# DaDaMrX/ReaLiSe

Measured on AMD Instinct MI355X. Metric: train sentences/sec (seq_len=128), higher is better.
Workload: dtype bf16

## Files before the change

### realise_amd/csrc/capi.hip

```cpp
#include <math.h>
#include <string.h>

#include "attention.h"
#include "engine.h"
#include "gemm.h"
#include "layout.h"
#include "ops.h"
#include "prof.h"
#include "../../include/realise_hip_debug.h"

using namespace rl;
#define RL_TRY(expr) do { const int _rc = (expr); if (_rc != RL_OK) return _rc; } while (0)

struct realise_engine { EngineBase* impl; };

namespace {
template <typename T> EpiParams<T> to_epi(const realise_epilogue* e) {
  EpiParams<T> p;
  if (!e) return p;
  p.mode = e->mode; p.accumulate = e->accumulate; p.out = (T*)e->out; p.ldo = e->ldo; p.out2 = (T*)e->out2;
  p.bias = e->bias; p.aux = (const T*)e->aux; p.ldaux = e->ldaux; p.alpha = e->alpha;
  p.drop_seed = e->drop_seed; p.drop_thresh = e->drop_thresh; p.drop_scale = e->drop_scale;
  return p;
}
// ... 124 lines not shown
  if (live == nullptr || n_live == nullptr) return RL_ERR_ARG;
  if (dtype == REALISE_BF16) return tn_grouped<bf16_t>(st, n, problems, P, live, n_live, list_rows, overwrite);
  if (dtype == REALISE_F32) return tn_grouped<float>(st, n, problems, P, live, n_live, list_rows, overwrite);
  return RL_ERR_ARG;
}
int realise_conv_tn(void* stream, int dtype, const void* A, int64_t lda, const realise_conv_geom* b, int P, int Co, int Ci,
                    float* out, float* scratch, int64_t scratch_elems) {
  hipStream_t st = (hipStream_t)stream;
  if (!b) return RL_ERR_ARG;
  TnEpi te; te.mode = TN_CONVW; te.out = out; te.Cin = Ci; te.Cpad = b->C; te.KHW = b->KH * b->KW;
  te.slab = scratch; te.slab_elems = scratch_elems;
  const int J = b->KH * b->KW * b->C;
  if (dtype == REALISE_BF16) return gemm_tn_conv<bf16_t>(st, (const bf16_t*)A, lda, to_geom<bf16_t>(b), P, Co, J, te);
  if (dtype == REALISE_F32) return gemm_tn_conv<float>(st, (const float*)A, lda, to_geom<float>(b), P, Co, J, te);
  return RL_ERR_ARG;
}
void realise_set_tn_transpose_read(int enable) { set_tn_transpose_read(enable); }
void realise_set_nt_allow_n96(int on) { set_nt_allow_n96(on); }
void realise_set_nt_variant(int v) { set_nt_variant(v); }
void realise_set_nt_group_m(int g) { set_nt8_group_m(g); }
void realise_set_ln(int key, int value) {
  if (key == 0) set_ln_fast(value); else if (key == 1) set_ln_bwd_blocks(value); else if (key == 2) set_bn_fast(value); else if (key == 3) set_bn_chunks(value); else if (key == 4) set_ce_fast(value); else if (key == 5) set_ln_v2(value); else if (key == 6) set_adamw_reg(value);
}
void realise_set_engine(int key, int value) { if (key == 0) set_fwd_order(value); else if (key >= 1 && key <= 3) set_stream_priority(key - 1, value); else if (key == 4) set_cls_compact(value); else if (key == 5) set_skip_dead(value); else if (key == 6) set_cls_splitk(value); else if (key == 9) set_gru_fuse(value); else if (key == 10) set_live_rows(value); else if (key == 13) set_glyph_fuse(value); else if (key == 14) set_bn_fold(value); else if (key == 15) set_opt_pipe(value); }
void realise_set_nt8p(int key, int value) { if (key == 0) set_nt8p_order(value); else if (key == 1) set_nt8p_wgs(value); else if (key == 3) set_nt8_live_gc(value); }
void realise_set_tn_split(int n) { set_tn_split(n); }
void realise_set_wgrad_group(int on) { set_wgrad_group(on); }
void realise_set_dgrad_parity(int on) { set_dgrad_parity(on); }
void realise_set_conv_c64(int on) { set_conv_c64(on); }
void realise_set_glyph_dedup(int on) { set_glyph_dedup(on); }
void realise_set_wgrad_overlap(int on) { set_wgrad_overlap(on); }
void realise_set_branch_overlap(int on) { set_branch_overlap(on); }

int realise_attention_fwd(void* stream, int dtype, const void* q, const void* k, const void* v, int64_t ldq, const float* mask_add,
                          void* ctx, int64_t ldc, float* lse, int B, int nh, int S, uint32_t drop_seed, uint32_t drop_thresh,
                          float drop_scale) {
  hipStream_t st = (hipStream_t)stream;
  if (dtype == REALISE_BF16)
    return attn_fwd<bf16_t>(st, (const bf16_t*)q, (const bf16_t*)k, (const bf16_t*)v, ldq, mask_add, (bf16_t*)ctx, ldc, lse, B, nh, S,
                            drop_seed, drop_thresh, drop_scale);
  if (dtype == REALISE_F32)
    return attn_fwd<float>(st, (const float*)q, (const float*)k, (const float*)v, ldq, mask_add, (float*)ctx, ldc, lse, B, nh, S,
                           drop_seed, drop_thresh, drop_scale);
  return RL_ERR_ARG;
}
int realise_attention_bwd(void* stream, int dtype, const void* q, const void* k, const void* v, int64_t ldq, const float* mask_add,
                          const void* ctx, const void* dctx, int64_t ldc, const float* lse, float* rowdot, void* dq, void* dk,
// ... 411 lines not shown
```

### realise_amd/csrc/engine.h

```cpp
#pragma once
#include <hip/hip_runtime.h>
#include <stdint.h>
#include "../../include/realise_hip.h"

namespace rl {
struct AdamwGroups;
void set_wgrad_overlap(int on);
void set_wgrad_group(int on);
void set_dgrad_parity(int on);
void set_fwd_order(int o);
void set_skip_dead(int on);
void set_cls_compact(int on);
void set_gru_fuse(int on);
void set_glyph_fuse(int on);
void set_opt_pipe(int on);
void set_bn_fold(int on);
void set_live_rows(int on);
void set_cls_splitk(int n);
void set_stream_priority(int which, int pri);
void set_branch_overlap(int on);

struct EngineBase {
  virtual ~EngineBase() {}
  virtual int64_t shadow_bytes() const = 0;
  virtual int64_t workspace_bytes(int B, int S, int Tp) = 0;
  virtual int bind(void* shadow, void* workspace, int64_t bytes) = 0;
  virtual void forget_workspace(void* workspace) = 0;
  virtual int64_t plan_install_count() const = 0;
  virtual int refresh_shadows(hipStream_t st) = 0;
  virtual int refresh_shadows_ex(hipStream_t st, int skip_linear) = 0;
  virtual int adamw_step(hipStream_t st, float* m, float* v, const uint8_t* group_of_block, const struct AdamwGroups& gs, const float* norm_sq,
                         float max_norm, int pipelined) = 0;
  virtual int sync_optimizer(hipStream_t st) = 0;
  virtual void invalidate_frozen() = 0;
  virtual void set_id_flag(int* flag) = 0;
  virtual void set_grads_fresh(int fresh) = 0;
  virtual void set_loss_grad(const float* grad_dev) = 0;
  virtual int forward(hipStream_t st, const realise_batch& b) = 0;
// ... 9 lines not shown
```

### realise_amd/csrc/engine.hip

```cpp
#include <math.h>
#include <stdio.h>
#include <string.h>
#include <algorithm>
#include <map>
#include <string>
#include <vector>

#include "attention.h"
#include "engine.h"
#include "gemm.h"
#include "layout.h"
#include "ops.h"

namespace rl {

static int g_wgrad_overlap = 1;
void set_wgrad_overlap(int on) { g_wgrad_overlap = on; }
static int g_wgrad_group = 1;
void set_wgrad_group(int on) { g_wgrad_group = on; }
static int g_dgrad_parity = 1;
void set_dgrad_parity(int on) { g_dgrad_parity = on; }
static int g_branch_overlap = 1;
void set_branch_overlap(int on) { g_branch_overlap = on; }
static int g_fwd_order = 0;
void set_fwd_order(int o) { g_fwd_order = o; }
static int g_skip_dead = 1;
void set_skip_dead(int on) { g_skip_dead = on; }
static int g_cls_compact = 1;
void set_cls_compact(int on) { g_cls_compact = on; }
static int g_gru_fuse = 1;
void set_gru_fuse(int on) { g_gru_fuse = on; }
static int g_cls_splitk = 3;
void set_cls_splitk(int n) { g_cls_splitk = n < 0 ? 0 : (n > 4 ? 4 : n); }
static int g_live_rows = 2;
void set_live_rows(int on) { g_live_rows = on; }
static int g_glyph_fuse = 1;
void set_glyph_fuse(int on) { g_glyph_fuse = on; }
static int g_bn_fold = 1;
void set_bn_fold(int on) { g_bn_fold = on; }
static int g_opt_pipe = 1;
void set_opt_pipe(int on) { g_opt_pipe = on; }
static int g_stream_pri[3] = {0, 0, 0};
void set_stream_priority(int which, int pri) { if (which >= 0 && which < 3) g_stream_pri[which] = pri < 0 ? -1 : (pri > 0 ? 1 : 0); }
static hipError_t create_stream(hipStream_t* s, int which) {
  if (g_stream_pri[which] == 0) return hipStreamCreateWithFlags(s, hipStreamNonBlocking);
  int least = 0, greatest = 0;
  if (hipDeviceGetStreamPriorityRange(&least, &greatest) != hipSuccess) return hipStreamCreateWithFlags(s, hipStreamNonBlocking);
  return hipStreamCreateWithPriority(s, hipStreamNonBlocking, g_stream_pri[which] < 0 ? greatest : least);
}

#define RL_TRY(expr) do { const int _rc = (expr); if (_rc != RL_OK) { fprintf(stderr, "[realise_hip] %s failed (%d) at %s:%d\n", #expr, _rc, __FILE__, __LINE__); return _rc; } } while (0)

static constexpr int64_t TN_SLAB_ELEMS = 16LL << 20;
static inline int64_t al256(int64_t x) { return (x + 255) & ~(int64_t)255; }
struct Bump {
  int64_t off = 0;
  int64_t take(int64_t bytes) { const int64_t o = off; off = al256(off + bytes); return o; }
};

static inline uint64_t splitmix(uint64_t x) {
  x += 0x9E3779B97F4A7C15ull;
  x = (x ^ (x >> 30)) * 0xBF58476D1CE4E5B9ull;
  x = (x ^ (x >> 27)) * 0x94D049BB133111EBull;
  return x ^ (x >> 31);
}

template <typename T> struct Engine : EngineBase {
  realise_config cfg;
  Variant vr;
  Layout L;
  float *P = nullptr, *G = nullptr, *PU = nullptr, *FZ = nullptr, *BF = nullptr;
  int64_t* BI = nullptr;
  char* sh = nullptr;
  char* ws = nullptr;
  int64_t ws_bytes = 0;
  int H, nh, I, V;
  int Vp;

  struct LayerSh { int64_t qkv_w, qkv_wT, ao_w, ao_wT, in_w, in_wT, out_w, out_wT; };
  struct BlockSh { int64_t w1f, w1d, w1p, w2f, w2d, wsf, wsd; int cin_pad; };
  std::vector<LayerSh> sh_bert, sh_pho, sh_out;
  BlockSh sh_blk[TOWER_MAX_BLOCKS];
  int64_t sh_cls_w = 0, sh_cls_wT = 0, sh_gru_hh = 0, sh_gru_hhT = 0, sh_glyph = 0;
  int64_t sh_head_w = 0, sh_head_wT = 0;
  int64_t shadow_total = 0;
  bool glyph_built = false, descs_built = false;
  int64_t sh_descs = 0, sh_fill = 0, sh_skip = 0;
  bool skip_built = false;
  static constexpr int ACHUNK_MAX = 8192, ACHUNK_LEN = 32768;
  std::vector<FillChunk> achunk_host;
  int n_achunks = 0;
  static constexpr int FILL_MAX = 2048;
  int n_descs = 0, desc_tiles = 0;
  std::vector<CastDesc> desc_host;

  struct LayerAct { int64_t qkv, lse, ctx, s1, rstd1, y1, pre, post, s2, rstd2, y2; };
  struct StackAct { int64_t emb_y, emb_xhat, emb_rstd; std::vector<LayerAct> layers; };
  struct BnAct { int64_t mean, rstd, scale, shift; };
  struct BlockAct { int64_t c1, h1, c2, cs, out; BnAct bn1, bn2, bns; int Hin, Hout, Pout; };
  struct Plan {
    int B = 0, S = 0, Tp = 0;
    int64_t total = 0;
    StackAct bert, pho, outb;
    BlockAct blk[TOWER_MAX_BLOCKS];
    int64_t mask_add, out_d, dlogits, count, loss_internal;
    int64_t cls_act, cls_inv, cls_nact, cls_xc, cls_gc, cls_slab;
    int64_t live_rows = 0;
    int64_t row_live, live_t64, live_t32, live_t16, live_n, live_rlen;
    int64_t ids_clean = 0, pho_clean = 0;
    int64_t gru_table, gru_hs, gru_rzn, gru_gh, gru_out;
    int64_t res_xhat, res_rstd, res_h, gate_mean, gate_msum, gate_g, fused;
// ... 164 lines not shown
    };
    auto add_stack = [&](const StackOff& so, const std::vector<LayerSh>& v) {
      for (size_t l = 0; l < v.size(); ++l) {
        const LayerOff& o = so.layers[l];
        add(o.qkv_w, 3 * H, H, v[l].qkv_w, v[l].qkv_wT);
        add(o.ao_w, H, H, v[l].ao_w, v[l].ao_wT);
        add(o.in_w, I, H, v[l].in_w, v[l].in_wT);
        add(o.out_w, H, I, v[l].out_w, v[l].out_wT);
      }
    };
    add_stack(L.bert, sh_bert);
    n_descs_a = (int)d.size(); desc_tiles_a = tiles;
    tiles = 0;
    add(L.cls_w, V, H, sh_cls_w, sh_cls_wT, Vp);
    if (vr.mlm_head) add(L.head_w, H, H, sh_head_w, sh_head_wT);
    if (vr.pho) add_stack(L.pho, sh_pho);
    if (vr.arch) add_stack(L.outb, sh_out);
    if (vr.pho) add(L.gru_w_hh, 3 * H, H, sh_gru_hh, sh_gru_hhT);
    if (d.size() > 256) return RL_ERR_ARG;
    if (hipMemcpyAsync(sh + sh_descs, d.data(), d.size() * sizeof(CastDesc), hipMemcpyHostToDevice, st) != hipSuccess) return RL_ERR_LAUNCH;
    n_descs = (int)d.size(); desc_tiles = tiles; descs_built = true;
    return RL_OK;
  }
  int refresh_shadows(hipStream_t st) override { return refresh_shadows_ex(st, 0); }
  int refresh_shadows_ex(hipStream_t st, int skip_linear) override {
    if (!sh) return RL_ERR_ARG;
    RL_TRY(ensure_descs(st));
    RL_TRY(wait_opt(st, skip_linear ? 0 : -1));
    if (!skip_linear) opt_pending = false;
    const bool ovl = vr.arch && branch_mask() != 0 && g_branch_overlap && branches_ok() && shadow_events_ok();
    hipStream_t s_b = ovl && vr.pho ? bst[0] : st, s_c = ovl && vr.res ? bst[1] : st;
    if (ovl) RL_TRY(fork(st));
    const CastDesc* dd = (const CastDesc*)(sh + sh_descs);
    if (!skip_linear) {
      RL_TRY(cast_transpose_multi<T>(st, dd, n_descs_a, desc_tiles_a));
      RL_TRY(cast_transpose_multi<T>(s_b, dd + n_descs_a, n_descs - n_descs_a, desc_tiles));
    }
    if (vr.res) {
      ConvShadowDescs cd;
      auto addc = [&](const float* w, int Co, int Ci, int KHW, int Cpad, T* fwd, T* dgrad, const TapOrder& ord = TapOrder()) {
        ConvShadowDesc& x = cd.d[cd.n++];
        x.w = w; x.fwd = fwd; x.dgrad = dgrad; x.Co = Co; x.Ci = Ci; x.KHW = KHW; x.Cpad = Cpad; x.CiRows = Cpad; x.block_begin = 0; x.order = ord;
      };
      for (int k = 0; k < L.tower.nblocks; ++k) {
        const BlockOff& o = L.blocks[k];
        const BlockSh& s = sh_blk[k];
        addc(pp(o.w1), o.cout, o.cin, 9, s.cin_pad, sp<T>(s.w1f), sp<T>(s.w1d));
        {
          TapOrder ord; ord.n = 9; int first = 0;
          (void)conv_s2_class(3, 3, 1, 0, &first, ord.t);
          addc(pp(o.w1), o.cout, o.cin, 9, s.cin_pad, (T*)nullptr, sp<T>(s.w1p), ord);
        }
        addc(pp(o.w2), o.cout, o.cout, 9, o.cout, sp<T>(s.w2f), sp<T>(s.w2d));
        addc(pp(o.ws), o.cout, o.cin, 1, s.cin_pad, sp<T>(s.wsf), sp<T>(s.wsd));
      }
      RL_TRY(conv_weight_shadow_multi<T>(s_c, cd));
      if (!glyph_built) {
        RL_TRY(glyph_shadow<T>(s_c, FZ + L.glyph, V, cfg.num_fonts, cfg.glyph_size * cfg.glyph_size, 8, sp<T>(sh_glyph)));
        glyph_built = true;
      }
    }
    shadows_pending = false;
    if (ovl) {
      for (int k = 0; k < 2; ++k) if ((branch_mask() >> k & 1) && hipEventRecord(ev_shadow[k], bst[k]) != hipSuccess) return RL_ERR_LAUNCH;
      shadows_pending = true;
    }
    return RL_OK;
  }
  static constexpr int OPT_EV_MAX = 16;
  hipEvent_t ev_opt[OPT_EV_MAX] = {}; hipEvent_t ev_grads = nullptr;
  int opt_groups = 0;
  bool opt_pending = false;
  bool opt_events_ok() {
    if (ev_grads != nullptr) return true;
    if (hipEventCreateWithFlags(&ev_grads, hipEventDisableTiming) != hipSuccess) { ev_grads = nullptr; return false; }
    for (int k = 0; k < OPT_EV_MAX; ++k)
      if (hipEventCreateWithFlags(&ev_opt[k], hipEventDisableTiming) != hipSuccess) return false;
    return true;
  }
  int wait_opt(hipStream_t s, int k) {
    if (!opt_pending) return RL_OK;
    if (g_opt_pipe >= 2) k = -1;
    const int lo = k < 0 ? 0 : std::min(k, opt_groups), hi = k < 0 ? opt_groups : lo;
    for (int i = lo; i <= hi; ++i) if (hipStreamWaitEvent(s, ev_opt[i], 0) != hipSuccess) return RL_ERR_LAUNCH;
    return RL_OK;
  }
  int sync_optimizer(hipStream_t st) override {
    RL_TRY(wait_opt(st, -1));
    opt_pending = false;
    return RL_OK;
  }
  int adamw_step(hipStream_t st, float* m, float* v, const uint8_t* group_of_block, const AdamwGroups& gs, const float* norm_sq,
                 float max_norm, int pipelined) override {
    if (!sh || !m || !v || !group_of_block) return RL_ERR_ARG;
    RL_TRY(ensure_descs(st));
    const int64_t n = L.arena_elems[AR_TRAIN];
    if (!skip_built) {
      std::vector<std::pair<int64_t, int64_t>> own;
      for (const CastDesc& d : desc_host) {
        const int64_t off = d.src - P, cnt = (int64_t)d.R * d.C;
        if ((off % 64) != 0 || (cnt % 64) != 0 || (d.C % 4) != 0) return RL_ERR_ARG;
        own.push_back({off, off + cnt});
      }
      std::sort(own.begin(), own.end());
      achunk_host.clear();
      int64_t at = 0;
      auto emit = [&](int64_t b, int64_t e) {
        for (int64_t o = b; o < e; o += ACHUNK_LEN) achunk_host.push_back(FillChunk{o, (int32_t)std::min<int64_t>(ACHUNK_LEN, e - o), 0});
      };
      for (auto& r : own) { if (r.first > at) emit(at, r.first); at = std::max(at, r.second); }
      if (at < n) emit(at, n);
      if ((int)achunk_host.size() > ACHUNK_MAX) return RL_ERR_ARG;
      if (!achunk_host.empty() &&
          hipMemcpyAsync(sh + sh_skip, achunk_host.data(), achunk_host.size() * sizeof(FillChunk), hipMemcpyHostToDevice, st) != hipSuccess) return RL_ERR_LAUNCH;
      n_achunks = (int)achunk_host.size();
      skip_built = true;
    }
    RL_TRY(wait_shadows(st));
    const CastDesc* dd = (const CastDesc*)(sh + sh_descs);
    RL_TRY(sync_optimizer(st));
    const int Lb = (int)sh_bert.size();
    if (pipelined && g_opt_pipe && side_ok() && opt_events_ok() && (Lb + 1) / 2 + 1 <= OPT_EV_MAX && n_descs_a == 4 * Lb) {
      RL_TRY(join_side(st));
      hipStream_t side = g_opt_pipe == 3 ? st : this->side;
      if (hipEventRecord(ev_grads, st) != hipSuccess || hipStreamWaitEvent(side, ev_grads, 0) != hipSuccess) return RL_ERR_LAUNCH;
      auto tile_begin = [&](int i, bool group_b) -> int {
        if (!group_b) return i < n_descs_a ? desc_host[i].tile_begin : desc_tiles_a;
        return n_descs_a + i < n_descs ? desc_host[n_descs_a + i].tile_begin : desc_tiles;
      };
      auto bert_layers = [&](int l0, int l1) -> int {
        const int a = 4 * l0, b = 4 * std::min(l1, Lb);
        if (b <= a) return RL_OK;
        return adamw_cast_multi<T>(side, dd + a, b - a, tile_begin(b, false) - tile_begin(a, false), P, G, m, v, group_of_block, gs, norm_sq, max_norm, tile_begin(a, false));
      };
      const int nb = n_descs - n_descs_a;
      const int nc = vr.mlm_head ? 2 : 1;
      opt_groups = (Lb + 1) / 2;
      RL_TRY(adamw_chunks(side, P, G, m, v, (const FillChunk*)(sh + sh_skip), n_achunks, group_of_block, gs, norm_sq, max_norm));
      RL_TRY(adamw_cast_multi<T>(side, dd + n_descs_a, nc, tile_begin(nc, true), P, G, m, v, group_of_block, gs, norm_sq, max_norm, 0));
      RL_TRY(bert_layers(0, 2));
      if (hipEventRecord(ev_opt[0], side) != hipSuccess) return RL_ERR_LAUNCH;
      for (int g = 1; g < opt_groups; ++g) {
        RL_TRY(bert_layers(2 * g, 2 * g + 2));
        if (hipEventRecord(ev_opt[g], side) != hipSuccess) return RL_ERR_LAUNCH;
        if (g == 1 && nb > nc) {
          RL_TRY(adamw_cast_multi<T>(side, dd + n_descs_a + nc, nb - nc, desc_tiles - tile_begin(nc, true), P, G, m, v, group_of_block, gs, norm_sq, max_norm, tile_begin(nc, true)));
          if (hipEventRecord(ev_opt[opt_groups], side) != hipSuccess) return RL_ERR_LAUNCH;
        }
      }
      if (opt_groups < 2 || nb <= nc) {
        if (opt_groups < 2 && nb > nc)
          RL_TRY(adamw_cast_multi<T>(side, dd + n_descs_a + nc, nb - nc, desc_tiles - tile_begin(nc, true), P, G, m, v, group_of_block, gs, norm_sq, max_norm, tile_begin(nc, true)));
        if (hipEventRecord(ev_opt[opt_groups], side) != hipSuccess) return RL_ERR_LAUNCH;
      }
      opt_pending = true;
      return RL_OK;
    }
    RL_TRY(adamw_cast_multi<T>(st, dd, n_descs_a, desc_tiles_a, P, G, m, v, group_of_block, gs, norm_sq, max_norm));
    RL_TRY(adamw_cast_multi<T>(st, dd + n_descs_a, n_descs - n_descs_a, desc_tiles, P, G, m, v, group_of_block, gs, norm_sq, max_norm));
    return adamw_chunks(st, P, G, m, v, (const FillChunk*)(sh + sh_skip), n_achunks, group_of_block, gs, norm_sq, max_norm);
  }
  hipEvent_t ev_shadow[2] = {nullptr, nullptr};
  bool shadows_pending = false;
  int n_descs_a = 0, desc_tiles_a = 0;
  bool shadow_events_ok() {
    for (int k = 0; k < 2; ++k)
      if (ev_shadow[k] == nullptr && hipEventCreateWithFlags(&ev_shadow[k], hipEventDisableTiming) != hipSuccess) return false;
    return true;
  }
  int wait_shadows(hipStream_t s) {
    if (!shadows_pending) return RL_OK;
    for (int k = 0; k < 2; ++k) if ((branch_mask() >> k & 1) && hipStreamWaitEvent(s, ev_shadow[k], 0) != hipSuccess) return RL_ERR_LAUNCH;
    return RL_OK;
  }

  void tap(const std::string& name, int64_t off, int64_t numel) { taps[name] = {off, numel}; }

  Plan make_plan(int B, int S, int Tp) {
    Plan p;
    const bool glyph_only = Tp < 0;
    p.B = B; p.S = S; p.Tp = Tp;
    Bump b;
// ... 130 lines not shown
    taps = keep;
    return p.total;
  }
  struct Slot { char* ws; int64_t bytes; Plan pl; std::map<std::string, std::pair<int64_t, int64_t>> taps; uint64_t stamp; };
  std::vector<Slot> slots;
  uint64_t slot_clock = 0;
  static constexpr size_t MAX_SLOTS = 8;
  void stash_current() {
    if (ws == nullptr) return;
    Slot* s = nullptr;
    for (Slot& x : slots) if (x.ws == ws) s = &x;
    if (s == nullptr) {
      if (slots.size() >= MAX_SLOTS) {
        size_t old = 0;
        for (size_t i = 1; i < slots.size(); ++i) if (slots[i].stamp < slots[old].stamp) old = i;
        slots.erase(slots.begin() + old);
      }
      slots.push_back(Slot());
      s = &slots.back();
    }
    s->ws = ws; s->bytes = ws_bytes; s->pl = pl; s->taps = taps; s->stamp = ++slot_clock;
  }
  int bind(void* shadow, void* workspace, int64_t bytes) override {
    if (shadow != (void*)sh) { glyph_built = false; descs_built = false; fill_built = false; n_fill = 0; skip_built = false; }
    stash_current();
    sh = (char*)shadow; ws = (char*)workspace; ws_bytes = bytes; pl = Plan(); have_fwd = false; have_glyph_fwd = false;
    for (Slot& x : slots)
      if (x.ws == ws && x.bytes == bytes) {
        pl = x.pl; taps = x.taps; x.stamp = ++slot_clock;
        break;
      }
    return RL_OK;
  }
  void forget_workspace(void* workspace) override {
    for (size_t i = 0; i < slots.size();) { if (slots[i].ws == (char*)workspace) slots.erase(slots.begin() + i); else ++i; }
    if (ws == (char*)workspace) { ws = nullptr; ws_bytes = 0; pl = Plan(); have_fwd = false; have_glyph_fwd = false; }
  }
  void invalidate_frozen() override { glyph_built = false; }
  int* id_flag = nullptr;
  void set_id_flag(int* flag) override { id_flag = flag; }
  int get_tap(const char* name, void** ptr, int64_t* numel) override {
    auto it = taps.find(name);
    if (it == taps.end() || !ws) return RL_ERR_ARG;
    *ptr = ws + it->second.first; *numel = it->second.second;
    return RL_OK;
  }

// ... 871 lines not shown
```

### realise_amd/csrc/ops.h

```cpp
#pragma once
#include "common.h"

namespace rl {

struct DropParams { uint32_t seed = 0, thresh = 0; float scale = 1.0f; };

constexpr int COL_SLOT_FLOATS = 262144;
constexpr int COL_SLOT_BYTES = COL_SLOT_FLOATS * 4;
constexpr int LN_SLOT_FLOATS = 1024 * 2 * 1024;
constexpr int LN_SLOT_BYTES = LN_SLOT_FLOATS * 4;
struct TapOrder { int n = 0; int t[9] = {0, 0, 0, 0, 0, 0, 0, 0, 0}; };

struct RowBound {
  const int* rows_dev = nullptr;
  const float* counts = nullptr;
  int hw = 1;
  float* slots = nullptr;
};
__device__ __forceinline__ int rb_rows(const RowBound& b, int P) { return b.rows_dev ? min(P, *b.rows_dev) : P; }
__device__ __forceinline__ float rb_weight(const RowBound& b, int row) { return b.counts ? b.counts[row / b.hw] : 1.0f; }

int mask_to_additive(hipStream_t st, const int64_t* masks, float* out, int n);
int sanitize_ids(hipStream_t st, const int64_t* ids, int64_t n, int V, int64_t* out, int* flag);

// ... 179 lines not shown
template <typename T> int cast_transpose(hipStream_t st, const float* src, int R, int C, T* dst, T* dstT);
struct CastDesc { const float* src; void* dst; void* dstT; int R, C; int tile_begin, tiles_c; int ldT; };
template <typename T> int cast_transpose_multi(hipStream_t st, const CastDesc* descs, int n, int total_tiles);
template <typename T>
int conv_weight_shadow(hipStream_t st, const float* w, int Co, int Ci, int KHW, int Cpad, int CiRows, T* fwd, T* dgrad, const TapOrder& order = TapOrder());
constexpr int CONV_SHADOW_MAX = 20;
struct ConvShadowDesc { const float* w; void* fwd; void* dgrad; int Co, Ci, KHW, Cpad, CiRows, block_begin; TapOrder order; };
struct ConvShadowDescs { int n = 0; ConvShadowDesc d[CONV_SHADOW_MAX]; };
template <typename T> int conv_weight_shadow_multi(hipStream_t st, ConvShadowDescs& ds);
template <typename T> int glyph_shadow(hipStream_t st, const float* tbl, int V, int F, int HW, int Cpad, T* out);

int sumsq_accum(hipStream_t st, const float* g, int64_t n, float* out);
int adamw_flat(hipStream_t st, float* p, const float* g, float* m, float* v, int64_t n, float lr, float beta1, float beta2,
               float eps, float weight_decay, float bias_c1, float bias_c2, const float* norm_sq, float max_norm);

constexpr int ADAMW_MAX_GROUPS = 8;
struct AdamwGroup { float lr, beta1, beta2, eps, weight_decay, step_size; };
struct AdamwGroups { int n; AdamwGroup g[ADAMW_MAX_GROUPS]; };
int adamw_grouped(hipStream_t st, float* p, const float* g, float* m, float* v, int64_t n, const uint8_t* group_of_block,
                  const AdamwGroups& gs, const float* norm_sq, float max_norm, const uint8_t* skip_block = nullptr);
template <typename T>
int adamw_cast_multi(hipStream_t st, const CastDesc* descs, int n, int total_tiles, float* P0, const float* G0, float* M0, float* V0,
                     const uint8_t* group_of_block, const AdamwGroups& gs, const float* norm_sq, float max_norm, int tile_base = 0);
int clip_scale(hipStream_t st, float* g, int64_t n, const float* norm_sq, float max_norm);
int fill_f32(hipStream_t st, float* p, float v, int64_t n);
struct FillChunk { int64_t off; int32_t len, pad; };
int zero_chunks(hipStream_t st, float* base, const FillChunk* chunks_dev, int n);
int adamw_chunks(hipStream_t st, float* p, const float* g, float* m, float* v, const FillChunk* chunks_dev, int n_chunks,
                 const uint8_t* group_of_block, const AdamwGroups& gs, const float* norm_sq, float max_norm);
int add_i64(hipStream_t st, int64_t* p, int64_t v, int n);

}
```

### realise_amd/csrc/ops2.hip

```cpp
#include <algorithm>
#include "ops.h"

namespace rl {

#define RL_LAUNCH_CHECK() (hipGetLastError() == hipSuccess ? RL_OK : RL_ERR_LAUNCH)

template <typename T>
__global__ void gru_step_fwd_kernel(GruStepArgs<T> a) {
  const int c = (blockIdx.x * blockDim.x + threadIdx.x) * 4;
  const int i = blockIdx.y;
  if (c >= a.H) return;
  if (a.n_alive_dev != nullptr && i >= *a.n_alive_dev) return;
  const int H = a.H;
  const int tok = a.perm[i];
  const int64_t v = a.pho_idx[(int64_t)tok * a.Tp + a.t];
  const float* gi = a.table + v * 3 * H + c;
  const floatx4 ir = *(const floatx4*)gi, iz = *(const floatx4*)(gi + H), in = *(const floatx4*)(gi + 2 * H);
  floatx4 hr, hz, hn, hp;
  if (a.gh != nullptr) {
    const T* gh = a.gh + (int64_t)i * 3 * H + c;
    hr = load4<T>(gh); hz = load4<T>(gh + H); hn = load4<T>(gh + 2 * H);
    hp = load4<T>(a.h_prev + (int64_t)i * H + c);
  } else {
    hr = *(const floatx4*)(a.b_hh + c); hz = *(const floatx4*)(a.b_hh + H + c); hn = *(const floatx4*)(a.b_hh + 2 * H + c);
// ... 633 lines not shown
    } else {
      if (dgrad == nullptr) continue;
      const int64_t k = i - nf;
      const int co = (int)(k % Co);
      const int tap = (int)((k / Co) % KHW);
      const int ci = (int)(k / ((int64_t)Co * KHW));
      const int src_tap = order.n ? order.t[tap] : tap;
      dgrad[k] = from_f<T>(ci < Ci ? w[((int64_t)co * Ci + ci) * KHW + src_tap] : 0.f);
    }
  }
}
template <typename T>
int conv_weight_shadow(hipStream_t st, const float* w, int Co, int Ci, int KHW, int Cpad, int CiRows, T* fwd, T* dgrad, const TapOrder& order) {
  if (order.n != 0 && order.n != KHW) return RL_ERR_ARG;
  const int64_t n = (int64_t)Co * KHW * Cpad + (int64_t)CiRows * KHW * Co;
  hipLaunchKernelGGL((conv_weight_shadow_kernel<T>), dim3(ew_blocks(n)), dim3(256), 0, st, w, Co, Ci, KHW, Cpad, CiRows, fwd, dgrad, order);
  return RL_LAUNCH_CHECK();
}
template int conv_weight_shadow<bf16_t>(hipStream_t, const float*, int, int, int, int, int, bf16_t*, bf16_t*, const TapOrder&);
template int conv_weight_shadow<float>(hipStream_t, const float*, int, int, int, int, int, float*, float*, const TapOrder&);

constexpr int CSH_T = 32;
template <typename T, int KHW, bool FULL>
__device__ __forceinline__ void conv_shadow_tile(const ConvShadowDesc& d, float (*tile)[CSH_T * 9 + 1], int co0, int ci0, int nco_, int nci_) {
  const int nco = FULL ? CSH_T : nco_, nci = FULL ? CSH_T : nci_, run = nci * KHW;
  const int Co = d.Co, Ci = d.Ci, Cpad = d.Cpad;
  T* fwd = (T*)d.fwd;
  T* dgrad = (T*)d.dgrad;
  for (int e = threadIdx.x; e < nco * run; e += 256) {
    const int c = e / run, r = e - c * run;
    tile[c][r] = d.w[((int64_t)(co0 + c) * Ci + ci0) * KHW + r];
  }
  __syncthreads();
  if (fwd != nullptr)
    for (int e = threadIdx.x; e < nco * KHW * nci; e += 256) {
      const int ci = e % nci, rest = e / nci, tap = rest % KHW, c = rest / KHW;
      fwd[((int64_t)(co0 + c) * KHW + tap) * Cpad + ci0 + ci] = from_f<T>(tile[c][ci * KHW + tap]);
    }
  if (dgrad != nullptr)
    for (int e = threadIdx.x; e < nci * KHW * nco; e += 256) {
      const int c = e % nco, rest = e / nco, slot = rest % KHW, ci = rest / KHW;
      const int src_tap = d.order.n ? d.order.t[slot] : slot;
      dgrad[((int64_t)(ci0 + ci) * KHW + slot) * Co + co0 + c] = from_f<T>(tile[c][ci * KHW + src_tap]);
    }
}
template <typename T>
__global__ void __launch_bounds__(256) conv_weight_shadow_multi_kernel(ConvShadowDescs ds) {
  __shared__ float tile[CSH_T][CSH_T * 9 + 1];
  int k = 0;
#pragma unroll 1
  for (int i = 1; i < ds.n; ++i) if ((int)blockIdx.x >= ds.d[i].block_begin) k = i;
  const ConvShadowDesc& d = ds.d[k];
  const int tiles_ci = (d.Ci + CSH_T - 1) / CSH_T;
  const int b = (int)blockIdx.x - d.block_begin;
  const int co0 = (b / tiles_ci) * CSH_T, ci0 = (b % tiles_ci) * CSH_T;
  const int nco = min(CSH_T, d.Co - co0), nci = min(CSH_T, d.Ci - ci0);
  const bool full = nco == CSH_T && nci == CSH_T;
  if (d.KHW == 9) { if (full) conv_shadow_tile<T, 9, true>(d, tile, co0, ci0, nco, nci); else conv_shadow_tile<T, 9, false>(d, tile, co0, ci0, nco, nci); }
  else if (d.KHW == 1) { if (full) conv_shadow_tile<T, 1, true>(d, tile, co0, ci0, nco, nci); else conv_shadow_tile<T, 1, false>(d, tile, co0, ci0, nco, nci); }
}
template <typename T> int conv_weight_shadow_multi(hipStream_t st, ConvShadowDescs& ds) {
  if (ds.n < 1 || ds.n > CONV_SHADOW_MAX) return RL_ERR_ARG;
  int blocks = 0;
  for (int k = 0; k < ds.n; ++k) {
    const ConvShadowDesc& d = ds.d[k];
    if ((d.order.n != 0 && d.order.n != d.KHW) || (d.KHW != 1 && d.KHW != 9) || d.Ci > d.Cpad || d.Ci > d.CiRows) return RL_ERR_ARG;
    ds.d[k].block_begin = blocks;
// ... 275 lines not shown
  if (dstT == nullptr) return;
#pragma unroll
  for (int j = 0; j < 4; ++j) {
    const floatx4 v = floatx4{pv[0][j], pv[1][j], pv[2][j], pv[3][j]};
    if (rb + 3 < d.R && (d.ldT & 3) == 0) store4<T>(dstT + (int64_t)(c + j) * d.ldT + rb, v);
    else for (int k = 0; k < 4 && rb + k < d.R; ++k) dstT[(int64_t)(c + j) * d.ldT + rb + k] = from_f<T>(v[k]);
  }
}
static int g_adamw_reg = 0;
void set_adamw_reg(int on) { g_adamw_reg = on; }

template <typename T>
int adamw_cast_multi(hipStream_t st, const CastDesc* descs, int n, int total_tiles, float* P0, const float* G0, float* M0, float* V0,
                     const uint8_t* group_of_block, const AdamwGroups& gs, const float* norm_sq, float max_norm, int tile_base) {
  if (n <= 0 || total_tiles <= 0) return RL_OK;
  if (gs.n < 1 || gs.n > ADAMW_MAX_GROUPS || group_of_block == nullptr) return RL_ERR_ARG;
  if (g_adamw_reg) hipLaunchKernelGGL((adamw_cast_multi_reg_kernel<T>), dim3(total_tiles), dim3(256), 0, st, descs, n, P0, G0, M0, V0, group_of_block, gs, norm_sq, max_norm, tile_base);
  else hipLaunchKernelGGL((adamw_cast_multi_kernel<T>), dim3(total_tiles), dim3(256), 0, st, descs, n, P0, G0, M0, V0, group_of_block, gs, norm_sq, max_norm, tile_base);
  return RL_LAUNCH_CHECK();
}
template int adamw_cast_multi<bf16_t>(hipStream_t, const CastDesc*, int, int, float*, const float*, float*, float*, const uint8_t*, const AdamwGroups&, const float*, float, int);
template int adamw_cast_multi<float>(hipStream_t, const CastDesc*, int, int, float*, const float*, float*, float*, const uint8_t*, const AdamwGroups&, const float*, float, int);

__global__ void clip_scale_kernel(float* __restrict__ g, int64_t n, const float* __restrict__ norm_sq, float max_norm) {
  const float c = max_norm / (sqrtf(norm_sq[0]) + 1e-6f);
  if (c >= 1.0f) return;
  for (int64_t i = (int64_t)blockIdx.x * blockDim.x + threadIdx.x; i < n; i += (int64_t)gridDim.x * blockDim.x) g[i] *= c;
}
int clip_scale(hipStream_t st, float* g, int64_t n, const float* norm_sq, float max_norm) {
  if (n <= 0) return RL_OK;
  hipLaunchKernelGGL(clip_scale_kernel, dim3(ew_blocks(n)), dim3(256), 0, st, g, n, norm_sq, max_norm);
  return RL_LAUNCH_CHECK();
}

__global__ void __launch_bounds__(256) zero_chunks_kernel(float* __restrict__ base, const FillChunk* __restrict__ chunks) {
  const FillChunk c = chunks[blockIdx.x];
  float* p = base + c.off;
  const int n4 = c.len >> 2;
  for (int i = threadIdx.x; i < n4; i += 256) ((floatx4*)p)[i] = floatx4{0.f, 0.f, 0.f, 0.f};
  for (int i = (n4 << 2) + threadIdx.x; i < c.len; i += 256) p[i] = 0.f;
}
int zero_chunks(hipStream_t st, float* base, const FillChunk* chunks_dev, int n) {
  if (n <= 0) return RL_OK;
  hipLaunchKernelGGL(zero_chunks_kernel, dim3(n), dim3(256), 0, st, base, chunks_dev);
  return RL_LAUNCH_CHECK();
}
// ... 20 lines not shown
```

Baseline: 4156.

## Fuse AdamW update of conv weights with bf16 conv shadow weight generation

Adds a kernel that applies the AdamW update to the conv tower weights tile by tile and, from the same shared-memory tile, writes the forward, dgrad and parity-ordered bf16 shadow copies. Those ranges are excluded from the generic AdamW chunk sweep, and the next refresh_shadows skips the separate conv shadow pass when the copies are already current. The aim is to avoid re-reading the fp32 conv weights and to drop one kernel launch per step. In exchange it adds state-tracking logic and moves the shadow-wait and optimizer sync earlier in adamw_step.

```diff
diff --git a/realise_amd/csrc/capi.hip b/realise_amd/csrc/capi.hip
--- a/realise_amd/csrc/capi.hip
+++ b/realise_amd/csrc/capi.hip
@@ -170,7 +170,7 @@
 void realise_set_ln(int key, int value) {
   if (key == 0) set_ln_fast(value); else if (key == 1) set_ln_bwd_blocks(value); else if (key == 2) set_bn_fast(value); else if (key == 3) set_bn_chunks(value); else if (key == 4) set_ce_fast(value); else if (key == 5) set_ln_v2(value); else if (key == 6) set_adamw_reg(value);
 }
-void realise_set_engine(int key, int value) { if (key == 0) set_fwd_order(value); else if (key >= 1 && key <= 3) set_stream_priority(key - 1, value); else if (key == 4) set_cls_compact(value); else if (key == 5) set_skip_dead(value); else if (key == 6) set_cls_splitk(value); else if (key == 9) set_gru_fuse(value); else if (key == 10) set_live_rows(value); else if (key == 13) set_glyph_fuse(value); else if (key == 14) set_bn_fold(value); else if (key == 15) set_opt_pipe(value); }
+void realise_set_engine(int key, int value) { if (key == 0) set_fwd_order(value); else if (key >= 1 && key <= 3) set_stream_priority(key - 1, value); else if (key == 4) set_cls_compact(value); else if (key == 5) set_skip_dead(value); else if (key == 6) set_cls_splitk(value); else if (key == 9) set_gru_fuse(value); else if (key == 10) set_live_rows(value); else if (key == 13) set_glyph_fuse(value); else if (key == 14) set_bn_fold(value); else if (key == 15) set_opt_pipe(value); else if (key == 16) set_conv_sweep(value); }
 void realise_set_nt8p(int key, int value) { if (key == 0) set_nt8p_order(value); else if (key == 1) set_nt8p_wgs(value); else if (key == 3) set_nt8_live_gc(value); }
 void realise_set_tn_split(int n) { set_tn_split(n); }
 void realise_set_wgrad_group(int on) { set_wgrad_group(on); }
diff --git a/realise_amd/csrc/engine.h b/realise_amd/csrc/engine.h
--- a/realise_amd/csrc/engine.h
+++ b/realise_amd/csrc/engine.h
@@ -14,6 +14,7 @@
 void set_gru_fuse(int on);
 void set_glyph_fuse(int on);
 void set_opt_pipe(int on);
+void set_conv_sweep(int on);
 void set_bn_fold(int on);
 void set_live_rows(int on);
 void set_cls_splitk(int n);
diff --git a/realise_amd/csrc/engine.hip b/realise_amd/csrc/engine.hip
--- a/realise_amd/csrc/engine.hip
+++ b/realise_amd/csrc/engine.hip
@@ -40,6 +40,8 @@
 void set_bn_fold(int on) { g_bn_fold = on; }
 static int g_opt_pipe = 1;
 void set_opt_pipe(int on) { g_opt_pipe = on; }
+static int g_conv_sweep = 1;
+void set_conv_sweep(int on) { g_conv_sweep = on; }
 static int g_stream_pri[3] = {0, 0, 0};
 void set_stream_priority(int which, int pri) { if (which >= 0 && which < 3) g_stream_pri[which] = pri < 0 ? -1 : (pri > 0 ? 1 : 0); }
 static hipError_t create_stream(hipStream_t* s, int which) {
@@ -86,7 +88,7 @@
   int64_t shadow_total = 0;
   bool glyph_built = false, descs_built = false;
   int64_t sh_descs = 0, sh_fill = 0, sh_skip = 0;
-  bool skip_built = false;
+  bool skip_built = false, skip_conv = false;
   static constexpr int ACHUNK_MAX = 8192, ACHUNK_LEN = 32768;
   std::vector<FillChunk> achunk_host;
   int n_achunks = 0;
@@ -297,6 +299,26 @@
     n_descs = (int)d.size(); desc_tiles = tiles; descs_built = true;
     return RL_OK;
   }
+  bool conv_copies_current = false;
+  void conv_descs(ConvSweepDescs& sd) const {
+    auto desc = [&](const float* w, int Co, int Ci, int KHW, int Cpad, T* fwd, T* dgrad, const TapOrder& ord = TapOrder()) {
+      ConvShadowDesc x;
+      x.w = w; x.fwd = fwd; x.dgrad = dgrad; x.Co = Co; x.Ci = Ci; x.KHW = KHW; x.Cpad = Cpad; x.CiRows = Cpad; x.block_begin = 0; x.order = ord;
+      return x;
+    };
+    const ConvShadowDesc none = desc(nullptr, 0, 0, 0, 0, nullptr, nullptr);
+    sd.n = 0;
+    for (int k = 0; k < L.tower.nblocks; ++k) {
+      const BlockOff& o = L.blocks[k];
+      const BlockSh& s = sh_blk[k];
+      TapOrder ord; ord.n = 9; int first = 0;
+      (void)conv_s2_class(3, 3, 1, 0, &first, ord.t);
+      sd.d[sd.n++] = ConvSweepDesc{desc(pp(o.w1), o.cout, o.cin, 9, s.cin_pad, sp<T>(s.w1f), sp<T>(s.w1d)),
+                                   desc(pp(o.w1), o.cout, o.cin, 9, s.cin_pad, (T*)nullptr, sp<T>(s.w1p), ord)};
+      sd.d[sd.n++] = ConvSweepDesc{desc(pp(o.w2), o.cout, o.cout, 9, o.cout, sp<T>(s.w2f), sp<T>(s.w2d)), none};
+      sd.d[sd.n++] = ConvSweepDesc{desc(pp(o.ws), o.cout, o.cin, 1, s.cin_pad, sp<T>(s.wsf), sp<T>(s.wsd)), none};
+    }
+  }
   int refresh_shadows(hipStream_t st) override { return refresh_shadows_ex(st, 0); }
   int refresh_shadows_ex(hipStream_t st, int skip_linear) override {
     if (!sh) return RL_ERR_ARG;
@@ -311,25 +333,19 @@
       RL_TRY(cast_transpose_multi<T>(st, dd, n_descs_a, desc_tiles_a));
       RL_TRY(cast_transpose_multi<T>(s_b, dd + n_descs_a, n_descs - n_descs_a, desc_tiles));
     }
+    const bool conv_current = skip_linear && conv_copies_current;
+    conv_copies_current = false;
     if (vr.res) {
-      ConvShadowDescs cd;
-      auto addc = [&](const float* w, int Co, int Ci, int KHW, int Cpad, T* fwd, T* dgrad, const TapOrder& ord = TapOrder()) {
-        ConvShadowDesc& x = cd.d[cd.n++];
-        x.w = w; x.fwd = fwd; x.dgrad = dgrad; x.Co = Co; x.Ci = Ci; x.KHW = KHW; x.Cpad = Cpad; x.CiRows = Cpad; x.block_begin = 0; x.order = ord;
-      };
-      for (int k = 0; k < L.tower.nblocks; ++k) {
-        const BlockOff& o = L.blocks[k];
-        const BlockSh& s = sh_blk[k];
-        addc(pp(o.w1), o.cout, o.cin, 9, s.cin_pad, sp<T>(s.w1f), sp<T>(s.w1d));
-        {
-          TapOrder ord; ord.n = 9; int first = 0;
-          (void)conv_s2_class(3, 3, 1, 0, &first, ord.t);
-          addc(pp(o.w1), o.cout, o.cin, 9, s.cin_pad, (T*)nullptr, sp<T>(s.w1p), ord);
+      if (!conv_current) {
+        ConvSweepDescs sd;
+        conv_descs(sd);
+        ConvShadowDescs cd;
+        for (int k = 0; k < sd.n; ++k) {
+          cd.d[cd.n++] = sd.d[k].a;
+          if (sd.d[k].b.dgrad != nullptr) cd.d[cd.n++] = sd.d[k].b;
         }
-        addc(pp(o.w2), o.cout, o.cout, 9, o.cout, sp<T>(s.w2f), sp<T>(s.w2d));
-        addc(pp(o.ws), o.cout, o.cin, 1, s.cin_pad, sp<T>(s.wsf), sp<T>(s.wsd));
-      }
-      RL_TRY(conv_weight_shadow_multi<T>(s_c, cd));
+        RL_TRY(conv_weight_shadow_multi<T>(s_c, cd));
+      }
       if (!glyph_built) {
         RL_TRY(glyph_shadow<T>(s_c, FZ + L.glyph, V, cfg.num_fonts, cfg.glyph_size * cfg.glyph_size, 8, sp<T>(sh_glyph)));
         glyph_built = true;
@@ -370,12 +386,28 @@
     if (!sh || !m || !v || !group_of_block) return RL_ERR_ARG;
     RL_TRY(ensure_descs(st));
     const int64_t n = L.arena_elems[AR_TRAIN];
-    if (!skip_built) {
+    RL_TRY(wait_shadows(st));
+    RL_TRY(sync_optimizer(st));
+    ConvSweepDescs csd;
+    bool conv_sweep = vr.res && g_conv_sweep != 0;
+    if (conv_sweep) {
+      conv_descs(csd);
+      for (int k = 0; k < csd.n; ++k) {
+        const ConvShadowDesc& a = csd.d[k].a;
+        if (((a.w - P) % 64) != 0 || ((int64_t)a.Co * a.Ci * a.KHW % 64) != 0) conv_sweep = false;
+      }
+    }
+    if (!conv_sweep) csd.n = 0;
+    if (!skip_built || skip_conv != conv_sweep) {
       std::vector<std::pair<int64_t, int64_t>> own;
       for (const CastDesc& d : desc_host) {
         const int64_t off = d.src - P, cnt = (int64_t)d.R * d.C;
         if ((off % 64) != 0 || (cnt % 64) != 0 || (d.C % 4) != 0) return RL_ERR_ARG;
         own.push_back({off, off + cnt});
+      }
+      for (int k = 0; k < csd.n; ++k) {
+        const ConvShadowDesc& a = csd.d[k].a;
+        own.push_back({a.w - P, a.w - P + (int64_t)a.Co * a.Ci * a.KHW});
       }
       std::sort(own.begin(), own.end());
       achunk_host.clear();
@@ -389,11 +421,10 @@
       if (!achunk_host.empty() &&
           hipMemcpyAsync(sh + sh_skip, achunk_host.data(), achunk_host.size() * sizeof(FillChunk), hipMemcpyHostToDevice, st) != hipSuccess) return RL_ERR_LAUNCH;
       n_achunks = (int)achunk_host.size();
-      skip_built = true;
-    }
-    RL_TRY(wait_shadows(st));
+      skip_built = true; skip_conv = conv_sweep;
+    }
     const CastDesc* dd = (const CastDesc*)(sh + sh_descs);
-    RL_TRY(sync_optimizer(st));
+    conv_copies_current = conv_sweep;
     const int Lb = (int)sh_bert.size();
     if (pipelined && g_opt_pipe && side_ok() && opt_events_ok() && (Lb + 1) / 2 + 1 <= OPT_EV_MAX && n_descs_a == 4 * Lb) {
       RL_TRY(join_side(st));
@@ -412,6 +443,7 @@
       const int nc = vr.mlm_head ? 2 : 1;
       opt_groups = (Lb + 1) / 2;
       RL_TRY(adamw_chunks(side, P, G, m, v, (const FillChunk*)(sh + sh_skip), n_achunks, group_of_block, gs, norm_sq, max_norm));
+      RL_TRY(adamw_conv_shadow_multi<T>(side, csd, P, G, m, v, n, group_of_block, gs, norm_sq, max_norm));
       RL_TRY(adamw_cast_multi<T>(side, dd + n_descs_a, nc, tile_begin(nc, true), P, G, m, v, group_of_block, gs, norm_sq, max_norm, 0));
       RL_TRY(bert_layers(0, 2));
       if (hipEventRecord(ev_opt[0], side) != hipSuccess) return RL_ERR_LAUNCH;
@@ -433,6 +465,7 @@
     }
     RL_TRY(adamw_cast_multi<T>(st, dd, n_descs_a, desc_tiles_a, P, G, m, v, group_of_block, gs, norm_sq, max_norm));
     RL_TRY(adamw_cast_multi<T>(st, dd + n_descs_a, n_descs - n_descs_a, desc_tiles, P, G, m, v, group_of_block, gs, norm_sq, max_norm));
+    RL_TRY(adamw_conv_shadow_multi<T>(st, csd, P, G, m, v, n, group_of_block, gs, norm_sq, max_norm));
     return adamw_chunks(st, P, G, m, v, (const FillChunk*)(sh + sh_skip), n_achunks, group_of_block, gs, norm_sq, max_norm);
   }
   hipEvent_t ev_shadow[2] = {nullptr, nullptr};
@@ -609,7 +642,7 @@
     s->ws = ws; s->bytes = ws_bytes; s->pl = pl; s->taps = taps; s->stamp = ++slot_clock;
   }
   int bind(void* shadow, void* workspace, int64_t bytes) override {
-    if (shadow != (void*)sh) { glyph_built = false; descs_built = false; fill_built = false; n_fill = 0; skip_built = false; }
+    if (shadow != (void*)sh) { glyph_built = false; descs_built = false; fill_built = false; n_fill = 0; skip_built = false; conv_copies_current = false; }
     stash_current();
     sh = (char*)shadow; ws = (char*)workspace; ws_bytes = bytes; pl = Plan(); have_fwd = false; have_glyph_fwd = false;
     for (Slot& x : slots)
diff --git a/realise_amd/csrc/ops.h b/realise_amd/csrc/ops.h
--- a/realise_amd/csrc/ops.h
+++ b/realise_amd/csrc/ops.h
@@ -225,6 +225,12 @@
 template <typename T>
 int adamw_cast_multi(hipStream_t st, const CastDesc* descs, int n, int total_tiles, float* P0, const float* G0, float* M0, float* V0,
                      const uint8_t* group_of_block, const AdamwGroups& gs, const float* norm_sq, float max_norm, int tile_base = 0);
+constexpr int CONV_SWEEP_MAX = 15;
+struct ConvSweepDesc { ConvShadowDesc a, b; };
+struct ConvSweepDescs { int n = 0; ConvSweepDesc d[CONV_SWEEP_MAX]; };
+template <typename T>
+int adamw_conv_shadow_multi(hipStream_t st, ConvSweepDescs& ds, float* P0, const float* G0, float* M0, float* V0, int64_t arena_elems,
+                            const uint8_t* group_of_block, const AdamwGroups& gs, const float* norm_sq, float max_norm);
 int clip_scale(hipStream_t st, float* g, int64_t n, const float* norm_sq, float max_norm);
 int fill_f32(hipStream_t st, float* p, float v, int64_t n);
 struct FillChunk { int64_t off; int32_t len, pad; };
diff --git a/realise_amd/csrc/ops2.hip b/realise_amd/csrc/ops2.hip
--- a/realise_amd/csrc/ops2.hip
+++ b/realise_amd/csrc/ops2.hip
@@ -679,16 +679,11 @@
 
 constexpr int CSH_T = 32;
 template <typename T, int KHW, bool FULL>
-__device__ __forceinline__ void conv_shadow_tile(const ConvShadowDesc& d, float (*tile)[CSH_T * 9 + 1], int co0, int ci0, int nco_, int nci_) {
-  const int nco = FULL ? CSH_T : nco_, nci = FULL ? CSH_T : nci_, run = nci * KHW;
-  const int Co = d.Co, Ci = d.Ci, Cpad = d.Cpad;
+__device__ __forceinline__ void conv_shadow_store(const ConvShadowDesc& d, float (*tile)[CSH_T * 9 + 1], int co0, int ci0, int nco_, int nci_) {
+  const int nco = FULL ? CSH_T : nco_, nci = FULL ? CSH_T : nci_;
+  const int Co = d.Co, Cpad = d.Cpad;
   T* fwd = (T*)d.fwd;
   T* dgrad = (T*)d.dgrad;
-  for (int e = threadIdx.x; e < nco * run; e += 256) {
-    const int c = e / run, r = e - c * run;
-    tile[c][r] = d.w[((int64_t)(co0 + c) * Ci + ci0) * KHW + r];
-  }
-  __syncthreads();
   if (fwd != nullptr)
     for (int e = threadIdx.x; e < nco * KHW * nci; e += 256) {
       const int ci = e % nci, rest = e / nci, tap = rest % KHW, c = rest / KHW;
@@ -700,6 +695,17 @@
       const int src_tap = d.order.n ? d.order.t[slot] : slot;
       dgrad[((int64_t)(ci0 + ci) * KHW + slot) * Co + co0 + c] = from_f<T>(tile[c][ci * KHW + src_tap]);
     }
+}
+template <typename T, int KHW, bool FULL>
+__device__ __forceinline__ void conv_shadow_tile(const ConvShadowDesc& d, float (*tile)[CSH_T * 9 + 1], int co0, int ci0, int nco_, int nci_) {
+  const int nco = FULL ? CSH_T : nco_, nci = FULL ? CSH_T : nci_, run = nci * KHW;
+  const int Ci = d.Ci;
+  for (int e = threadIdx.x; e < nco * run; e += 256) {
+    const int c = e / run, r = e - c * run;
+    tile[c][r] = d.w[((int64_t)(co0 + c) * Ci + ci0) * KHW + r];
+  }
+  __syncthreads();
+  conv_shadow_store<T, KHW, FULL>(d, tile, co0, ci0, nco_, nci_);
 }
 template <typename T>
 __global__ void __launch_bounds__(256) conv_weight_shadow_multi_kernel(ConvShadowDescs ds) {
@@ -1021,6 +1027,110 @@
 template int adamw_cast_multi<bf16_t>(hipStream_t, const CastDesc*, int, int, float*, const float*, float*, float*, const uint8_t*, const AdamwGroups&, const float*, float, int);
 template int adamw_cast_multi<float>(hipStream_t, const CastDesc*, int, int, float*, const float*, float*, float*, const uint8_t*, const AdamwGroups&, const float*, float, int);
 
+template <typename T, int KHW, bool FULL>
+__device__ __forceinline__ void adamw_conv_tile(const ConvSweepDesc& d, float (*tile)[CSH_T * 9 + 1], int co0, int ci0, int nco_, int nci_,
+                                                float* __restrict__ P0, const float* __restrict__ G0, float* __restrict__ M0, float* __restrict__ V0,
+                                                const uint8_t* __restrict__ group_of_block, const AdamwGroups& gs, float clip) {
+  const int nco = FULL ? CSH_T : nco_, nci = FULL ? CSH_T : nci_, run = nci * KHW;
+  const int Ci = d.a.Ci;
+  const int64_t base = d.a.w - P0;
+  if (FULL && (Ci & 3) == 0) {
+    constexpr int RQ = CSH_T * KHW / 4;
+    for (int qd = threadIdx.x; qd < CSH_T * RQ; qd += 256) {
+      const int c = qd / RQ, r = (qd - c * RQ) * 4;
+      const int64_t e = base + ((int64_t)(co0 + c) * Ci + ci0) * KHW + r;
+      floatx4 pv = *(const floatx4*)(P0 + e);
+      const int gid = group_of_block[e >> 6];
+      if (gid < gs.n) {
+        const AdamwGroup h = gs.g[gid];
+        floatx4 mv = *(const floatx4*)(M0 + e), vv = *(const floatx4*)(V0 + e);
+        const floatx4 gv = *(const floatx4*)(G0 + e) * clip;
+#pragma unroll
+        for (int j = 0; j < 4; ++j) {
+          mv[j] = mv[j] * h.beta1 + (1.0f - h.beta1) * gv[j];
+          vv[j] = vv[j] * h.beta2 + (1.0f - h.beta2) * gv[j] * gv[j];
+          float pi = pv[j] - h.step_size * (mv[j] / (sqrtf(vv[j]) + h.eps));
+          if (h.weight_decay > 0.f) pi -= h.lr * h.weight_decay * pi;
+          pv[j] = pi;
+        }
+        *(floatx4*)(M0 + e) = mv; *(floatx4*)(V0 + e) = vv; *(floatx4*)(P0 + e) = pv;
+      }
+#pragma unroll
+      for (int j = 0; j < 4; ++j) tile[c][r + j] = pv[j];
+    }
+  } else {
+    for (int k = threadIdx.x; k < nco * run; k += 256) {
+      const int c = k / run, r = k - c * run;
+      const int64_t e = base + ((int64_t)(co0 + c) * Ci + ci0) * KHW + r;
+      float pi = P0[e];
+      const int gid = group_of_block[e >> 6];
+      if (gid < gs.n) {
+        const AdamwGroup h = gs.g[gid];
+        const float gi = G0[e] * clip;
+        const float mi = M0[e] * h.beta1 + (1.0f - h.beta1) * gi;
+        const float vi = V0[e] * h.beta2 + (1.0f - h.beta2) * gi * gi;
+        pi = pi - h.step_size * (mi / (sqrtf(vi) + h.eps));
+        if (h.weight_decay > 0.f) pi -= h.lr * h.weight_decay * pi;
+        M0[e] = mi; V0[e] = vi; P0[e] = pi;
+      }
+      tile[c][r] = pi;
+    }
+  }
+  __syncthreads();
+  conv_shadow_store<T, KHW, FULL>(d.a, tile, co0, ci0, nco_, nci_);
+  if (d.b.dgrad != nullptr) conv_shadow_store<T, KHW, FULL>(d.b, tile, co0, ci0, nco_, nci_);
+}
+template <typename T>
+__global__ void __launch_bounds__(256) adamw_conv_shadow_multi_kernel(ConvSweepDescs ds, float* __restrict__ P0, const float* __restrict__ G0,
+                                                                      float* __restrict__ M0, float* __restrict__ V0,
+                                                                      const uint8_t* __restrict__ group_of_block, AdamwGroups gs,
+                                                                      const float* __restrict__ norm_sq, float max_norm) {
+  __shared__ float tile[CSH_T][CSH_T * 9 + 1];
+  int k = 0;
+#pragma unroll 1
+  for (int i = 1; i < ds.n; ++i) if ((int)blockIdx.x >= ds.d[i].a.block_begin) k = i;
+  const ConvSweepDesc& d = ds.d[k];
+  const int tiles_ci = (d.a.Ci + CSH_T - 1) / CSH_T;
+  const int b = (int)blockIdx.x - d.a.block_begin;
+  const int co0 = (b / tiles_ci) * CSH_T, ci0 = (b % tiles_ci) * CSH_T;
+  const int nco = min(CSH_T, d.a.Co - co0), nci = min(CSH_T, d.a.Ci - ci0);
+  const bool full = nco == CSH_T && nci == CSH_T;
+  float clip = 1.0f;
+  if (norm_sq != nullptr) {
+    const float c = max_norm / (sqrtf(norm_sq[0]) + 1e-6f);
+    clip = c < 1.0f ? c : 1.0f;
+  }
+  if (d.a.KHW == 9) {
+    if (full) adamw_conv_tile<T, 9, true>(d, tile, co0, ci0, nco, nci, P0, G0, M0, V0, group_of_block, gs, clip);
+    else adamw_conv_tile<T, 9, false>(d, tile, co0, ci0, nco, nci, P0, G0, M0, V0, group_of_block, gs, clip);
+  } else if (d.a.KHW == 1) {
+    if (full) adamw_conv_tile<T, 1, true>(d, tile, co0, ci0, nco, nci, P0, G0, M0, V0, group_of_block, gs, clip);
+    else adamw_conv_tile<T, 1, false>(d, tile, co0, ci0, nco, nci, P0, G0, M0, V0, group_of_block, gs, clip);
+  }
+}
+template <typename T>
+int adamw_conv_shadow_multi(hipStream_t st, ConvSweepDescs& ds, float* P0, const float* G0, float* M0, float* V0, int64_t arena_elems,
+                            const uint8_t* group_of_block, const AdamwGroups& gs, const float* norm_sq, float max_norm) {
+  if (ds.n == 0) return RL_OK;
+  if (ds.n < 0 || ds.n > CONV_SWEEP_MAX) return RL_ERR_ARG;
+  if (gs.n < 1 || gs.n > ADAMW_MAX_GROUPS || group_of_block == nullptr) return RL_ERR_ARG;
+  int blocks = 0;
+  for (int k = 0; k < ds.n; ++k) {
+    const ConvShadowDesc& a = ds.d[k].a;
+    const ConvShadowDesc& b = ds.d[k].b;
+    if ((a.order.n != 0 && a.order.n != a.KHW) || (a.KHW != 1 && a.KHW != 9) || a.Ci > a.Cpad || a.Ci > a.CiRows) return RL_ERR_ARG;
+    if (b.dgrad != nullptr && (b.fwd != nullptr || b.Co != a.Co || b.Ci != a.Ci || b.KHW != a.KHW || b.order.n != a.KHW || b.Ci > b.CiRows)) return RL_ERR_ARG;
+    const int64_t off = a.w - P0, cnt = (int64_t)a.Co * a.Ci * a.KHW;
+    if (off < 0 || (off & 63) != 0 || off + cnt > arena_elems) return RL_ERR_ARG;
+    ds.d[k].a.block_begin = blocks;
+    blocks += ((a.Co + CSH_T - 1) / CSH_T) * ((a.Ci + CSH_T - 1) / CSH_T);
+  }
+  hipLaunchKernelGGL((adamw_conv_shadow_multi_kernel<T>), dim3(blocks), dim3(256), 0, st, ds, P0, G0, M0, V0, group_of_block, gs, norm_sq, max_norm);
+  return RL_LAUNCH_CHECK();
+}
+template int adamw_conv_shadow_multi<bf16_t>(hipStream_t, ConvSweepDescs&, float*, const float*, float*, float*, int64_t, const uint8_t*, const AdamwGroups&, const float*, float);
+template int adamw_conv_shadow_multi<float>(hipStream_t, ConvSweepDescs&, float*, const float*, float*, float*, int64_t, const uint8_t*, const AdamwGroups&, const float*, float);
+
 __global__ void clip_scale_kernel(float* __restrict__ g, int64_t n, const float* __restrict__ norm_sq, float max_norm) {
   const float c = max_norm / (sqrtf(norm_sq[0]) + 1e-6f);
   if (c >= 1.0f) return;
```

Result: no change. 4138 (-0.4%).
